# Autobot37/weatherforecastingtoolkit

Hardware: AMD Instinct MI355X
Metric: SEVIR 384x384 frames/sec (AE train step) (higher is better)
Workload: dtype f32; 1 GPU; experiments/ae_v2 conv AE (ae_64x8x8_lin.PosAwareAE_TF, img_size=384), 1x384x384 synthetic SEVIR frames, batch 32/GPU, fp32, fwd + L1 + bwd + AdamW + cosine-warmup LR; batch_per_gpu=32, global_batch=32, img_size=384, parallelism=dp1, params=215033281

## Files before the change

### include/wfae.h

```cpp
#ifndef WFAE_H
#define WFAE_H

#include <stddef.h>
#include <stdint.h>

#ifdef __cplusplus
extern "C" {
#endif

typedef void* wfae_stream_t;

typedef enum {
  WFAE_OK = 0,
  WFAE_ERR_BAD_SHAPE = -1,
  WFAE_ERR_NULL_POINTER = -2,
  WFAE_ERR_WORKSPACE = -3,
  WFAE_ERR_LAUNCH = -4,
  WFAE_ERR_UNSUPPORTED = -5
} wfae_status;

int wfae_version(void);
const char* wfae_last_error_string(void);
size_t wfae_workspace_bytes(int64_t max_weight_elems);

// ... 4 lines not shown
int wfae_set_split_gemm(int on);
int wfae_get_split_gemm(void);

int wfae_set_c1n(int on);
int wfae_get_c1n(void);

int wfae_conv1x1_fwd(const float* x, const float* w, const float* bias, const float* res,
                     int64_t res_img_stride, float* y, int NB, int Cin, int Cout, int HW,
                     wfae_stream_t stream);
int wfae_conv1x1_fwd_stats(const float* x, const float* w, const float* bias, const float* res,
                           int64_t res_img_stride, float* y, int NB, int Cin, int Cout, int HW,
                           double* stat_part, int64_t stat_capacity, int* stat_rows, wfae_stream_t stream);
int wfae_conv1x1_fwd_bnact(const float* x, const float* bn_scale, const float* bn_shift, const float* w,
                           const float* bias, const float* res, int64_t res_img_stride, float* y, int NB, int Cin,
                           int Cout, int HW, double* stat_part, int64_t stat_capacity, int* stat_rows,
                           wfae_stream_t stream);
int wfae_conv1x1_bwd_weight_bnact(const float* dy, const float* x, const float* bn_scale, const float* bn_shift,
                                  float* dw, int NB, int Cin, int Cout, int HW, int accumulate, void* ws,
                                  size_t ws_bytes, wfae_stream_t stream);
int wfae_conv1x1_bwd_data(const float* dy, const float* w, float* dx, int NB, int Cin, int Cout,
                          int HW, wfae_stream_t stream);
int wfae_conv1x1_bwd_weight(const float* dy, const float* x, float* dw, int NB, int Cin, int Cout,
                            int HW, int accumulate, void* ws, size_t ws_bytes, wfae_stream_t stream);

int wfae_c1r_supported(int M, int K, int HW);
int wfae_c1r_stat_rows(int M, int K, int NB, int HW);
int wfae_c1r_fwd(const float* w, int64_t w_sm, int64_t w_sk, const float* x, const float* pro_scale, const float* pro_shift,
                 const float* res, float* y, int NB, int K, int M, int HW, double* stat_part, int64_t stat_capacity,
                 int* stat_rows, wfae_stream_t stream);
int wfae_c1r_bnred_supported(int M, int K, int HW);
int wfae_c1r_bnred(const float* w, int64_t w_sm, int64_t w_sk, const float* dt, const float* x, const float* bn_scale,
                   const float* bn_shift, const float* save_mean, const float* save_invstd, float* da, int NB, int K, int M, int HW,
                   double* part, int64_t part_capacity, int* part_rows, wfae_stream_t stream);
int wfae_bn_act_bwd_from_rows(const double* part, int rows, int C, float* dgamma, float* dbeta, int accumulate, void* ws,
                              size_t ws_bytes, wfae_stream_t stream);
int wfae_c1r_bndx(const float* w, int64_t w_sm, int64_t w_sk, const float* dt, const float* x, const float* gamma,
                  const float* bn_scale, const float* bn_shift, const float* save_mean, const float* save_invstd, const float* coef,
                  const float* res, float* dx, int NB, int K, int M, int HW, int training, wfae_stream_t stream);
int wfae_c1rb_supported(int M, int K, int HW);
int wfae_c1rb_stat_rows(int M, int K, int NB, int HW);
int wfae_c1rb_fwd(const float* w, int64_t w_sm, int64_t w_sk, const uint16_t* x, const float* pro_scale, const float* pro_shift,
                  const uint16_t* res, uint16_t* y, int NB, int K, int M, int HW, double* stat_part, int64_t stat_capacity,
                  int* stat_rows, wfae_stream_t stream);
int wfae_c1w_supported(int Cin, int Cout, int HW);
int wfae_c1w_bwd_weight(const float* dy, const float* x, const float* bn_scale, const float* bn_shift, float* dw, int NB, int Cin,
                        int Cout, int HW, int accumulate, void* ws, size_t ws_bytes, wfae_stream_t stream);
int wfae_c1w_bwd_weight_bf16(const uint16_t* dy, const uint16_t* x, const float* bn_scale, const float* bn_shift, float* dw, int NB,
                             int Cin, int Cout, int HW, int accumulate, void* ws, size_t ws_bytes, wfae_stream_t stream);
int wfae_set_c1wd(int on);
int wfae_get_c1wd(void);
int wfae_c1wd_supported(int C, int mid, int HW);
int wfae_c1wd_bwd(const float* dy, const float* t2, const float* bn_scale, const float* bn_shift, const float* w3, float* dw3,
                  float* da3, int NB, int C, int mid, int HW, int accumulate, void* ws, size_t ws_bytes, wfae_stream_t stream);
int wfae_set_c1ws(int on);
int wfae_get_c1ws(void);
int wfae_c1ws_supported(int C, int mid, int HW);
int wfae_c1ws_stat_rows(int C, int mid, int NB, int HW, size_t ws_bytes);
int wfae_c1ws_bwd(const float* x, const float* dt1, const float* bn_scale, const float* bn_shift, const float* save_mean,
                  const float* save_invstd, const float* w1, float* dw1, double* part, int64_t part_capacity, int* part_rows, int NB,
                  int C, int mid, int HW, int accumulate, void* ws, size_t ws_bytes, wfae_stream_t stream);
int wfae_linear_fwd(const float* x, const float* w, const float* bias, float* y, int B, int In,
                    int Out, void* ws, size_t ws_bytes, wfae_stream_t stream);
int wfae_linear_bwd_data(const float* dy, const float* w, float* dx, int B, int In, int Out,
                         wfae_stream_t stream);
int wfae_linear_bwd_weight(const float* dy, const float* x, float* dw, int B, int In, int Out,
                           int accumulate, wfae_stream_t stream);
int wfae_linear_bwd_data_splitk(const float* dy, const float* w, float* dx, int B, int In, int Out, void* ws,
                                size_t ws_bytes, wfae_stream_t stream);
int wfae_linear_bwd_weight_splitk(const float* dy, const float* x, float* dw, int B, int In, int Out, int accumulate,
                                  void* ws, size_t ws_bytes, wfae_stream_t stream);

int wfae_conv4x4s2_down(const float* hi, const float* w, float* lo, int NB, int Chi, int Clo,
                        int Hlo, int Wlo, wfae_stream_t stream);
int wfae_conv4x4s2_up(const float* lo, const float* w, float* hi, int NB, int Chi, int Clo, int Hlo,
                      int Wlo, void* ws, size_t ws_bytes, wfae_stream_t stream);
int wfae_conv4x4s2_wgrad(const float* lo, const float* hi, float* dw, int NB, int Chi, int Clo,
                         int Hlo, int Wlo, int accumulate, void* ws, size_t ws_bytes,
                         wfae_stream_t stream);

int wfae_dconv_fwd(const float* x, const float* w, const float* bias, float* y, int NB, int Cin,
                   int Cout, int H, int W, int KS, int stride, int pad, int groups,
                   wfae_stream_t stream);
int wfae_dconv_bwd_data(const float* dy, const float* w, float* dx, int NB, int Cin, int Cout,
                        int H, int W, int KS, int pad, int groups, wfae_stream_t stream);
int wfae_dconv_bwd_weight(const float* dy, const float* x, float* dw, int NB, int Cin, int Cout,
                          int H, int W, int KS, int stride, int pad, int groups, int accumulate,
                          void* ws, size_t ws_bytes, wfae_stream_t stream);

int wfae_gconv3x3_fwd(const float* x, const float* w, float* y, int NB, int C, int H, int W, int groups,
                      int transposed, void* ws, size_t ws_bytes, wfae_stream_t stream);
int wfae_gconv3x3_bwd_weight(const float* dy, const float* x, float* dw, int NB, int C, int H, int W,
                             int groups, int accumulate, void* ws, size_t ws_bytes, wfae_stream_t stream);

int wfae_bn_stats_train(const float* x, int NB, int C, int HW, const float* gamma,
                        const float* beta, float eps, float momentum, float* running_mean,
                        float* running_var, float* save_mean, float* save_invstd, float* scale,
                        float* shift, void* ws, size_t ws_bytes, wfae_stream_t stream);
int wfae_bn_stats_from_rows(const double* stat_part, int rows, int NB, int C, int HW, const float* gamma,
                            const float* beta, float eps, float momentum, float* running_mean,
                            float* running_var, float* save_mean, float* save_invstd, float* scale,
                            float* shift, void* ws, size_t ws_bytes, wfae_stream_t stream);
int wfae_bn_fold_eval(const float* gamma, const float* beta, const float* running_mean,
                      const float* running_var, float eps, float* save_mean, float* save_invstd,
                      float* scale, float* shift, int C, wfae_stream_t stream);
int wfae_bn_act_fwd(const float* x, const float* scale, const float* shift, float* y, int NB, int C,
                    int HW, int act, wfae_stream_t stream);
// ... 359 lines not shown
```

### weatherforecastingtoolkit_amd/csrc/c1wd.hip

```cpp
#include "common.h"
#include <atomic>
#include <stdlib.h>
#include <type_traits>

using namespace wfae;

namespace {

typedef float f32x4 __attribute__((ext_vector_type(4)));
typedef float f32x16 __attribute__((ext_vector_type(16)));
typedef __bf16 bf16x8 __attribute__((ext_vector_type(8)));
typedef short s16x4 __attribute__((ext_vector_type(4)));
typedef short s16x8 __attribute__((ext_vector_type(8)));
typedef unsigned u32x4 __attribute__((ext_vector_type(4)));
typedef unsigned u32x2 __attribute__((ext_vector_type(2)));

struct C1WDP {
  const float* dy;
  const float* t2;
  const float* w3;
  const float* pro_scale;
  const float* pro_shift;
  float* slab;
  float* da;
  int HW;
  int cpi;
  int kc;
};

constexpr int DNT = 512, DBK = 32;

__device__ __forceinline__ unsigned off_row(int r, int c) { return (unsigned)(r * 64 + ((c ^ ((r >> 2) & 3)) << 4)); }

__device__ __forceinline__ void split_pair(float a, float b, unsigned& h, unsigned& m, unsigned& l) {
  h = pack_bf16(a, b);
  const float ra = a - bf16_lo(h), rb = b - bf16_hi(h);
  m = pack_bf16(ra, rb);
  l = pack_bf16(ra - bf16_lo(m), rb - bf16_hi(m));
}

template <int C>
__global__ __launch_bounds__(DNT, C == 128 ? 4 : 2) void c1wd_kernel(C1WDP p) {
  constexpr int M = C / 4;
  constexpr int TM = C / 128;
  constexpr int WQ = M / 32;
  constexpr int NDW = 4 * WQ;
  constexpr bool BOTH = NDW == 8;
  constexpr int KCH = C / 32;
  constexpr int LPR = 8;
  constexpr int P_LD = C * LPR, Q_LD = M * LPR;
  constexpr int P_IT = P_LD / DNT;
  static_assert(P_LD % DNT == 0 && Q_LD <= DNT, "loader");
  constexpr int A_PLANE_B = C * 64, B_PLANE_B = M * 64;
  constexpr int A_STAGE_B = 3 * A_PLANE_B, STAGE_B = 3 * (A_PLANE_B + B_PLANE_B);
  __shared__ __attribute__((aligned(16))) unsigned char smem[2 * STAGE_B];
  const int t = threadIdx.x, lane = t & 63;
  const int wave = __builtin_amdgcn_readfirstlane(t >> 6);
  const int img = blockIdx.x / p.cpi, chunk = blockIdx.x - img * p.cpi;
  const int k_begin = chunk * p.kc;
  const int k_end = min(p.HW, k_begin + p.kc);
  const int nsteps = (k_end - k_begin) / DBK;
  const bool do_dw = BOTH || wave < NDW, do_da = BOTH || wave >= NDW;

  const float* Pb = p.dy + (long)img * C * p.HW + k_begin;
  const float* Qb = p.t2 + (long)img * M * p.HW + k_begin;
  const float* p_src[P_IT];
  unsigned p_dst[P_IT];
#pragma unroll
  for (int j = 0; j < P_IT; ++j) {
    const int idx = t + j * DNT, r = idx / LPR, e = idx % LPR;
    p_src[j] = Pb + (long)r * p.HW + e * 4;
    p_dst[j] = off_row(r, e >> 1) + (unsigned)((e & 1) * 8);
  }
  const bool q_on = Q_LD == DNT || t < Q_LD;
  const int q_r = q_on ? t / LPR : 0, q_e = t % LPR;
  const float* q_src = Qb + (long)q_r * p.HW + q_e * 4;
  const unsigned q_dst = off_row(q_r, q_e >> 1) + (unsigned)((q_e & 1) * 8);
  const float q_s = p.pro_scale[q_r], q_h = p.pro_shift[q_r];
  u32x4 rp[P_IT], rq;
  auto load_global = [&]() {
#pragma unroll
    for (int j = 0; j < P_IT; ++j) rp[j] = *reinterpret_cast<const u32x4*>(p_src[j]);
    if (q_on) rq = *reinterpret_cast<const u32x4*>(q_src);
  };
  auto advance = [&](bool more) {
#pragma unroll
    for (int j = 0; j < P_IT; ++j) p_src[j] += more ? DBK : 0;
    q_src += more ? DBK : 0;
  };
  auto put = [&](unsigned char* base, int plane_b, unsigned dst, u32x4 r, bool act, float s, float h) {
    const unsigned u0 = r[0], u1 = r[1], u2 = r[2], u3 = r[3];
    float v0 = __uint_as_float(u0), v1 = __uint_as_float(u1), v2 = __uint_as_float(u2), v3 = __uint_as_float(u3);
    if (act) {
      v0 = gelu_f(fmaf(v0, s, h)); v1 = gelu_f(fmaf(v1, s, h));
      v2 = gelu_f(fmaf(v2, s, h)); v3 = gelu_f(fmaf(v3, s, h));
    }
    unsigned h0, m0, l0, h1, m1, l1;
    split_pair(v0, v1, h0, m0, l0);
    split_pair(v2, v3, h1, m1, l1);
    *reinterpret_cast<u32x2*>(base + dst) = u32x2{h0, h1};
    *reinterpret_cast<u32x2*>(base + plane_b + dst) = u32x2{m0, m1};
    *reinterpret_cast<u32x2*>(base + 2 * plane_b + dst) = u32x2{l0, l1};
  };
  auto store_lds = [&](int buf) {
    unsigned char* s = smem + buf * STAGE_B;
#pragma unroll
    for (int j = 0; j < P_IT; ++j) put(s, A_PLANE_B, p_dst[j], rp[j], false, 0.f, 0.f);
    if (q_on) put(s + A_STAGE_B, B_PLANE_B, q_dst, rq, true, q_s, q_h);
  };

  const int wm0 = (BOTH ? (wave >> 1) : (wave & 3)) * (32 * TM), wn0 = BOTH ? (wave & 1) * 32 : 0;
  const int r31 = lane & 31, lh = lane >> 5;
  const unsigned a_rd = (unsigned)((wm0 + r31) * 64), b_rd = (unsigned)((wn0 + r31) * 64);
  const int a_x = (r31 >> 2) & 3;
  f32x16 acc[TM];
  struct Frag {
    bf16x8 a[TM][3], b[3];
  };
  auto read_frag = [&](Frag& f, int buf, int ks) {
    const unsigned char* s = smem + buf * STAGE_B;
    const unsigned a_c = (unsigned)(((2 * ks + lh) ^ a_x) << 4);
#pragma unroll
    for (int i = 0; i < TM; ++i)
#pragma unroll
      for (int pl = 0; pl < 3; ++pl)
        f.a[i][pl] = *reinterpret_cast<const bf16x8*>(s + pl * A_PLANE_B + a_rd + i * (32 * 64) + a_c);
#pragma unroll
    for (int pl = 0; pl < 3; ++pl) f.b[pl] = *reinterpret_cast<const bf16x8*>(s + A_STAGE_B + pl * B_PLANE_B + b_rd + a_c);
  };
  auto mfma_frag = [&](const Frag& f) {
#pragma unroll
    for (int i = 0; i < TM; ++i) {
      f32x16 c = acc[i];
      c = __builtin_amdgcn_mfma_f32_32x32x16_bf16(f.a[i][2], f.b[0], c, 0, 0, 0);
      c = __builtin_amdgcn_mfma_f32_32x32x16_bf16(f.a[i][0], f.b[2], c, 0, 0, 0);
      c = __builtin_amdgcn_mfma_f32_32x32x16_bf16(f.a[i][1], f.b[1], c, 0, 0, 0);
      c = __builtin_amdgcn_mfma_f32_32x32x16_bf16(f.a[i][1], f.b[0], c, 0, 0, 0);
      c = __builtin_amdgcn_mfma_f32_32x32x16_bf16(f.a[i][0], f.b[1], c, 0, 0, 0);
      c = __builtin_amdgcn_mfma_f32_32x32x16_bf16(f.a[i][0], f.b[0], c, 0, 0, 0);
      acc[i] = c;
    }
  };

  const int dtile = BOTH ? wave : (wave & 3);
  const int mt = dtile >> 1, pt = dtile & 1;
  const int n16 = lane & 15, kg = lane >> 4, tq = n16 >> 2, tp = n16 & 3;
  bf16x8 wa[KCH][3];
  auto load_weights = [&]() {
#pragma unroll
    for (int ch = 0; ch < KCH; ++ch) {
      const float* src = p.w3 + (long)(32 * ch + 8 * kg) * M + 16 * mt + n16;
      float v[8];
#pragma unroll
      for (int e = 0; e < 8; ++e) v[e] = src[e * M];
      u32x4 h, m, l;
#pragma unroll
      for (int e = 0; e < 4; ++e) {
        unsigned qh, qm, ql;
        split_pair(v[2 * e], v[2 * e + 1], qh, qm, ql);
        h[e] = qh; m[e] = qm; l[e] = ql;
      }
      wa[ch][0] = __builtin_bit_cast(bf16x8, h);
      wa[ch][1] = __builtin_bit_cast(bf16x8, m);
      wa[ch][2] = __builtin_bit_cast(bf16x8, l);
    }
  };
  unsigned tr_rd[2];
#pragma unroll
  for (int hf = 0; hf < 2; ++hf) tr_rd[hf] = off_row(8 * kg + 4 * hf + tq, 2 * pt + (tp >> 1)) + 8u * (unsigned)(tp & 1);
  float* const da_dst = p.da + ((long)img * M + 16 * mt + 4 * kg) * p.HW + k_begin + 16 * pt + n16;
  auto da_step = [&](int buf, int st) {
    const unsigned char* s = smem + buf * STAGE_B;
    constexpr int PA[6] = {2, 0, 1, 1, 0, 0}, PB[6] = {0, 2, 1, 0, 1, 0};
    f32x4 d = {0.f, 0.f, 0.f, 0.f};
#pragma unroll
    for (int ch = 0; ch < KCH; ++ch) {
      bf16x8 b[3];
#pragma unroll
      for (int pl = 0; pl < 3; ++pl) {
        s16x4 part[2];
#pragma unroll
        for (int hf = 0; hf < 2; ++hf)
          part[hf] = __builtin_amdgcn_ds_read_tr16_b64_v4i16(
              (s16x4 __attribute__((address_space(3)))*)(s + pl * A_PLANE_B + ch * (32 * 64) + tr_rd[hf]));
        b[pl] = __builtin_bit_cast(bf16x8, __builtin_shufflevector(part[0], part[1], 0, 1, 2, 3, 4, 5, 6, 7));
      }
#pragma unroll
      for (int pr = 0; pr < 6; ++pr) d = __builtin_amdgcn_mfma_f32_16x16x32_bf16(wa[ch][PA[pr]], b[PB[pr]], d, 0, 0, 0);
    }
    float* o = da_dst + 32 * st;
#pragma unroll
    for (int q = 0; q < 4; ++q) o[(long)q * p.HW] = d[q];
  };

  auto run = [&](auto dwc, auto dac) {
    constexpr bool DW = decltype(dwc)::value, DA = decltype(dac)::value;
    if constexpr (DW) {
#pragma unroll
      for (int i = 0; i < TM; ++i)
#pragma unroll
        for (int q = 0; q < 16; ++q) acc[i][q] = 0.f;
    }
    if constexpr (DA) load_weights();
    if (nsteps > 0) {
      Frag f0, f1;
      load_global();
      advance(nsteps > 1);
      store_lds(0);
      load_global();
      advance(nsteps > 2);
      __syncthreads();
      if constexpr (DW) read_frag(f0, 0, 0);
      for (int st = 0; st < nsteps; ++st) {
        const int cur = st & 1;
        if constexpr (DW) read_frag(f1, cur, 1);
        store_lds(cur ^ 1);
        load_global();
        advance(st + 3 < nsteps);
        if constexpr (DW) mfma_frag(f0);
        if constexpr (DA) da_step(cur, st);
        __builtin_amdgcn_sched_barrier(0);
        __syncthreads();
        __builtin_amdgcn_sched_barrier(0);
        if constexpr (DW) {
          read_frag(f0, cur ^ 1, 0);
          mfma_frag(f1);
        }
        __builtin_amdgcn_sched_barrier(0);
      }
    }
    if constexpr (DW) {
      float* __restrict__ Cb = p.slab + (long)blockIdx.x * C * M;
#pragma unroll
      for (int i = 0; i < TM; ++i)
#pragma unroll
        for (int q = 0; q < 16; ++q) {
          const int row = wm0 + 32 * i + (q & 3) + 8 * (q >> 2) + 4 * lh;
          Cb[(long)row * M + wn0 + r31] = acc[i][q];
        }
    }
  };
  if constexpr (BOTH) run(std::true_type{}, std::true_type{});
  else if (do_dw) run(std::true_type{}, std::false_type{});
  else run(std::false_type{}, std::true_type{});
}

std::atomic<int> g_c1wd{-1};
inline bool c1wd_on() {
  int v = g_c1wd.load(std::memory_order_relaxed);
  if (v < 0) {
    const char* e = getenv("WFAE_C1WD");
    v = (e && e[0] == '0') ? 0 : 1;
    g_c1wd.store(v, std::memory_order_relaxed);
  }
  return v == 1;
}

inline bool al16(const void* q) { return (reinterpret_cast<uintptr_t>(q) & 15) == 0; }

inline bool c1wd_shape_ok(int C, int mid, int HW) { return (C == 128 || C == 256) && mid * 4 == C && HW > 0 && HW % 64 == 0; }

}

extern "C" {

int wfae_set_c1wd(int on) {
  g_c1wd.store(on ? 1 : 0, std::memory_order_relaxed);
  return WFAE_OK;
}

int wfae_get_c1wd(void) { return c1wd_on() ? 1 : 0; }

int wfae_c1wd_supported(int C, int mid, int HW) {
  return (c1wd_on() && c1wd_shape_ok(C, mid, HW) && wfae::split_gemm_enabled()) ? 1 : 0;
}

int wfae_c1wd_bwd(const float* dy, const float* t2, const float* bn_scale, const float* bn_shift, const float* w3, float* dw3,
                  float* da3, int NB, int C, int mid, int HW, int accumulate, void* ws, size_t ws_bytes, wfae_stream_t stream) {
  WFAE_REQUIRE(dy && t2 && bn_scale && bn_shift && w3 && dw3 && da3 && ws, WFAE_ERR_NULL_POINTER, "c1wd_bwd: null pointer");
  WFAE_REQUIRE(NB > 0 && C > 0 && mid > 0 && HW > 0 && NB <= 65535 && (int64_t)NB * HW < (1ll << 31), WFAE_ERR_BAD_SHAPE,
               "c1wd_bwd: bad shape");
  WFAE_REQUIRE(c1wd_shape_ok(C, mid, HW), WFAE_ERR_UNSUPPORTED,
               "c1wd_bwd: serves C = 128 or 256 with mid = C / 4 and HW %% 64 == 0 (C %d, mid %d, HW %d)", C, mid, HW);
  WFAE_REQUIRE(c1wd_on() && wfae::split_gemm_enabled(), WFAE_ERR_UNSUPPORTED,
               "c1wd_bwd: needs fp32 precision with the split GEMMs on and wfae_set_c1wd(1)");
  WFAE_REQUIRE(al16(dy) && al16(t2), WFAE_ERR_UNSUPPORTED, "c1wd_bwd: dy and t2 must be 16-byte aligned");
  C1WDP p = {};
  p.dy = dy; p.t2 = t2; p.w3 = w3;
  p.pro_scale = bn_scale; p.pro_shift = bn_shift;
  p.slab = (float*)ws; p.da = da3;
  p.HW = HW;
  WFAE_REQUIRE(c1w_chunks(C, mid, NB, HW, ws_bytes, &p.cpi, &p.kc), WFAE_ERR_WORKSPACE, "c1wd_bwd: workspace %zu < %zu", ws_bytes,
               (size_t)NB * C * mid * sizeof(float));
  hipStream_t st = (hipStream_t)stream;
  const dim3 grid((unsigned)(NB * p.cpi)), block(DNT);
  if (C == 128) hipLaunchKernelGGL((c1wd_kernel<128>), grid, block, 0, st, p);
  else hipLaunchKernelGGL((c1wd_kernel<256>), grid, block, 0, st, p);
  const int rc = check_launch("c1wd_bwd");
  if (rc) return rc;
  return slab_reduce((const float*)ws, dw3, nullptr, (long)C * mid, mid, NB * p.cpi, accumulate, st, 0);
}

}
```

### weatherforecastingtoolkit_amd/functional.py

```python
from __future__ import annotations

import os

import torch
from torch.autograd import Function

from . import ops

BN_EPS = 1e-5


_overlap = False
_side = {}


STAT_FUSION = os.environ.get("WFAE_STAT_FUSION", "1") == "1"


FUSE_A1 = os.environ.get("WFAE_FUSE_A1", "1") == "1"
FUSE_A1_MAXC = 1 << 30
FUSE_A3 = os.environ.get("WFAE_FUSE_A3", "1") == "1"
FUSE_A3_MAXC = int(os.environ.get("WFAE_FUSE_A3_MAXC", "128"))
FUSE_A3_MAXC_C1R = max(FUSE_A3_MAXC, 256)

# ... 471 lines not shown
class BottleneckFn(Function):
    @staticmethod
    def forward(ctx, x, g1, b1, w1, g2, b2, wg, g3, b3, w3, mod, x_stats=None):
        xc = _c(x)
        if xc is not x:
            x_stats = None
        x = xc
        bn1, bn2, bn3 = mod.f[0], mod.f[3], mod.f[6]
        groups = mod.f[5].groups
        training = _use_batch_stats(bn1)
        fuse = training and STAT_FUSION
        emit = fuse and getattr(mod, "emit_stats", False)
        C, mid, hw = x.shape[1], w1.shape[0], x.shape[2] * x.shape[3]
        sto = _storage(x)

        def route(op, m, k, pro=False, res="none"):
            return ops.conv1x1_route(op, m, k, hw, sto, pro, False, res)
        fused1 = FUSE_A1 and C <= FUSE_A1_MAXC and ops.conv1x1_bnact_supported(x, mid)
        r1, r3 = route("fwd", mid, C, fused1), route("fwd", C, mid, True, "ordinary")
        fused3 = (FUSE_A3 and C <= (FUSE_A3_MAXC_C1R if r3 in ("c1r", "c1rb") else FUSE_A3_MAXC)
                  and ops.conv1x1_bnact_supported((x.shape[0], mid) + x.shape[2:], C))
        if not fused3:
            r3 = route("fwd", C, mid, False, "ordinary")
        d1, d3 = (route("dgrad", C, mid), route("dgrad", mid, C)) if sto == "bf16" else (None, None)
        W1p, W3p = (ops.c1b_weights(w1), ops.c1b_weights(w3)) if "c1b" in (r1, r3, d1, d3) else ((None, None), (None, None))
        st1 = _bn_stats_rows(x_stats if (fuse or isinstance(x_stats, ops.StatParts)) else None, x, bn1, training)
        a1 = None if fused1 else ops.bn_act_fwd(x, st1, 1)
        t1, sr2 = _c1(w1, W1p[0], False, *((x, st1) if fused1 else (a1, None)), None, fuse, r1)
        st2 = _bn_stats_rows(sr2, t1, bn2, training)
        a2 = ops.bn_act_fwd(t1, st2, 1)
        t2 = _g3_fwd(a2, wg, groups)
        st3 = _bn_stats(t2, bn3, training)
        a3 = None if fused3 else ops.bn_act_fwd(t2, st3, 1)
        y, mod._out_stats = _c1(w3, W3p[0], False, *((t2, st3) if fused3 else (a3, None)), x, emit, r3)
        ctx.save_for_backward(x, _opt(a1), t1, a2, t2, _opt(a3), g1, w1, g2, wg, g3, w3,
                              st1.mean, st1.invstd, st1.scale, st1.shift,
                              st2.mean, st2.invstd, st2.scale, st2.shift,
                              st3.mean, st3.invstd, st3.scale, st3.shift,
                              _opt(W1p[1] if d1 == "c1b" else None), _opt(W3p[1] if d3 == "c1b" else None))
        ctx.training = training
        ctx.groups = groups
        ctx.betas = (b1, b2, b3)
        return y

    @staticmethod
    def backward(ctx, dy):
        (x, a1, t1, a2, t2, a3, g1, w1, g2, wg, g3, w3, *s) = ctx.saved_tensors
        st1, st2, st3 = _mk_stats(*s[0:4]), _mk_stats(*s[4:8]), _mk_stats(*s[8:12])
        W1t, W3t = s[12], s[13]
        tr = ctx.training
        dy = _c(dy)
        mid = w1.shape[0]
        dw3 = grad_buffer(w3)
        da3 = None
        if a3.numel() == 0:
            if ops.conv1x1_wd_route(dy.shape[1], mid, dy.shape[2] * dy.shape[3], _storage(dy)) == "c1wd":
                da3 = _on_main(lambda: ops.conv1x1_bwd_wd(dy, t2, st3, w3, dw3))
            if da3 is None:
                _wgrad(lambda: ops.conv1x1_bwd_weight_bnact(dy, t2, st3, dw3), dy, t2, st3.scale, st3.shift)
        else:
            _wgrad(lambda: ops.conv1x1_bwd_weight(dy, a3, dw3), dy, a3)
        dg3, db3 = grad_buffer(g3), grad_buffer(ctx.betas[2])
        if da3 is not None:
            dt2 = ops.bn_act_bwd(da3, t2, g3, st3, dg3, db3, None, 1, tr)
        else:
            dt2 = _dgrad_bn(dy, w3, W3t, t2, g3, st3, dg3, db3, None, tr)
        del da3
        dwg = grad_buffer(wg)
        _wgrad(lambda: _g3_wgrad(dt2, a2, dwg, ctx.groups), dt2, a2)
        da2 = _g3_dgrad(dt2, wg, mid, ctx.groups)
        del dt2
        dg2, db2 = grad_buffer(g2), grad_buffer(ctx.betas[1])
        dt1 = ops.bn_act_bwd(da2, t1, g2, st2, dg2, db2, None, 1, tr)
        del da2
        dw1 = grad_buffer(w1)
        rows1 = None
        if a1.numel() == 0:
            if ops.conv1x1_ws_route(x.shape[1], mid, x.shape[2] * x.shape[3], _storage(x)) == "c1ws":
                rows1 = _on_main(lambda: ops.conv1x1_bwd_ws(dt1, x, st1, w1, dw1))
            if rows1 is None:
                _wgrad(lambda: ops.conv1x1_bwd_weight_bnact(dt1, x, st1, dw1), dt1, x, st1.scale, st1.shift)
        else:
            _wgrad(lambda: ops.conv1x1_bwd_weight(dt1, a1, dw1), dt1, a1)
        dg1, db1 = grad_buffer(g1), grad_buffer(ctx.betas[0])
        dx = _dgrad_bn(dt1, w1, W1t, x, g1, st1, dg1, db1, dy, tr, rows1)
        return dx, dg1, db1, dw1, dg2, db2, dwg, dg3, db3, dw3, None, None


class Conv1x1Fn(Function):

    @staticmethod
    def forward(ctx, x, w, bias, pos):
        ctx.x_dtype = x.dtype
        x = ops.to_f32(_c(x))
        y = ops.conv1x1_fwd(x, w, bias, None if pos is None else _c(pos), pos is not None)
        ctx.save_for_backward(x, w)
        ctx.bias, ctx.pos = bias, pos
        return y

    @staticmethod
    def backward(ctx, dy):
        x, w = ctx.saved_tensors
        dy = ops.to_f32(_c(dy))
        nb, cout, h, wd = dy.shape
        dw = grad_buffer(w)
        ops.conv1x1_bwd_weight(dy, x, dw)
        dx = ops.to_dtype(ops.conv1x1_bwd_data(dy, w), ctx.x_dtype) if ctx.needs_input_grad[0] else None
        dbias = dpos = None
        if ctx.bias is not None:
            dbias = grad_buffer(ctx.bias)
            ops.reduce_sum(dy, nb, cout, h * wd, dbias)
        if ctx.pos is not None:
            dpos = grad_buffer(ctx.pos)
            ops.reduce_sum(dy, nb, cout * h * wd, 1, dpos)
        return dx, dw, dbias, dpos

# ... 1034 lines not shown
```

### weatherforecastingtoolkit_amd/ops.py

```python
from __future__ import annotations

import ctypes
import math
import os

import torch

from . import _lib

_WS_DEFAULT = int(os.environ.get("WFAE_WORKSPACE_MB", "512")) << 20
_ws = {}


def _stream():
    return torch.cuda.current_stream().cuda_stream


_prof = None


def profile_start():
    global _prof
    _prof = {}

# ... 159 lines not shown
def _p(t):
    return None if t is None else t.data_ptr()


class StatRows:
    __slots__ = ("part", "rows")

    def __init__(self, part, rows):
        self.part, self.rows = part, rows


class StatParts:
    __slots__ = ("part", "splits")

    def __init__(self, part, splits):
        self.part, self.splits = part, splits


def _rows_out(n, device):
    part = torch.empty(n, dtype=torch.float64, device=device)
    count = ctypes.c_int(0)
    return part, count, (part.data_ptr(), n, ctypes.cast(ctypes.pointer(count), ctypes.c_void_p))


_NO_ROWS = (None, 0, None)


_C1R = _C1R_BNRED = _C1R_BNDX = _C1RB = _C1B = _C1W = True


def set_c1r(on):
    global _C1R
    _C1R = bool(on)


def set_c1r_bnred(on):
    global _C1R_BNRED
    _C1R_BNRED = bool(on)


def set_c1r_bndx(on):
    global _C1R_BNDX
    _C1R_BNDX = bool(on)


def set_c1n(on):
    _lib.call("wfae_set_c1n", int(bool(on)))


def set_c1wd(on):
    _lib.call("wfae_set_c1wd", int(bool(on)))


def set_c1ws(on):
    _lib.call("wfae_set_c1ws", int(bool(on)))


def set_c1rb(on):
    global _C1RB
    _C1RB = bool(on)


def set_c1b(on):
    global _C1B
    _C1B = bool(on)


def set_c1w(on):
    global _C1W
    _C1W = bool(on)


def c1r_bndx_on():
    return _C1R_BNDX


def c1n_enabled():
    return bool(_lib.load().wfae_get_c1n())


def c1wd_enabled():
    return bool(_lib.load().wfae_get_c1wd())


def c1ws_enabled():
    return bool(_lib.load().wfae_get_c1ws())


def _precision():
    return _lib.load().wfae_get_matmul_precision()


def c1r_supported(m, k, hw):
    return _C1R and _SPLIT_GEMM and _precision() == 0 and bool(_lib.load().wfae_c1r_supported(int(m), int(k), int(hw)))


def c1r_bnred_supported(m, k, hw):
    return (_C1R and _C1R_BNRED and _SPLIT_GEMM and _precision() == 0
            and bool(_lib.load().wfae_c1r_bnred_supported(int(m), int(k), int(hw))))


def c1rb_supported(m, k, hw):
    return _C1RB and _precision() == 1 and bool(_lib.load().wfae_c1rb_supported(int(m), int(k), int(hw)))


def c1b_supported(m, k, hw):
    return _C1B and _precision() == 1 and bool(_lib.load().wfae_c1b_supported(int(m), int(k), int(hw)))


def conv1x1_bnact_supported(x, cout):
    nb, cin, h, wd = getattr(x, "shape", x)
    swapped = cin < cout and cin < 128
    return (h * wd) % 4 == 0 and h * wd >= 16 and cin % 4 == 0 and (cout % 4 == 0 or not swapped)


def conv1x1_route(op, m, k, hw, storage="f32", prologue=False, bias=False, residual="none"):
    if op == "wgrad":
        ok = _C1W and _lib.load().wfae_c1w_supported(int(k), int(m), int(hw))
        return "c1w" if ok and (_precision() == 1 if storage == "bf16" else (_precision() == 0 and _SPLIT_GEMM)) else "gemm"
    if bias or residual == "broadcast" or (residual == "ordinary" and m <= k):
        return "gemm"
    if storage == "f32":
        return "c1r" if c1r_supported(m, k, hw) else "gemm"
    rb = c1rb_supported(m, k, hw)
    if rb and not (prologue and m < k and k >= 256):
        return "c1rb"
    return "c1b" if (rb or c1b_supported(m, k, hw)) else "gemm"


def conv1x1_dgrad_bn_route(m, k, hw, storage="f32"):
    if storage == "f32" and c1r_bnred_supported(m, k, hw):
        return "bndx" if _C1R_BNDX else "bnred"
    return None


# ... 91 lines not shown
    _chk(w)
    cout, cin = w.shape[0], w.shape[1]
    Wb = torch.empty((cout, cin), dtype=BF16, device=w.device)
    Wtb = torch.empty((cin, cout), dtype=BF16, device=w.device)
    _call("wfae_c1b_weights", 0, 8 * w.numel(), _p(w), _p(Wb), _p(Wtb), cout, cin, _stream())
    return Wb, Wtb


def c1b_fwd(Wb, x, st=None, res=None, stats=False, label="wfae_c1b_fwd"):
    r = _c1_launch("c1b", Wb, False, x, st, None, res, False, stats, label)
    return r if stats else r[0]


def _c1_wgrad(dy, x, st, dw, accumulate):
    sfx, es = _chka(dy, x)
    _chk(dw)
    nb, cout, h, wd = dy.shape
    cin, n = x.shape[1], nb * h * wd
    pro = (None, None) if st is None else (_p(st.scale), _p(st.shift))
    peak = None
    if conv1x1_route("wgrad", cout, cin, h * wd, "bf16" if sfx else "f32", st is not None) == "c1w":
        name, peak = "wfae_c1w_bwd_weight" + sfx, PEAK_BF16_MFMA / (1 if sfx else 6)
    elif sfx:
        name = "wfae_conv1x1_bwd_weight_bf16"
    else:
        name, pro = ("wfae_conv1x1_bwd_weight", ()) if st is None else ("wfae_conv1x1_bwd_weight_bnact", pro)
    ws = workspace()
    _call(name, 2 * n * cin * cout, es * n * (cin + cout) + 4 * cin * cout, _p(dy), _p(x), *pro, _p(dw), nb, cin, cout, h * wd,
          int(accumulate), ws.data_ptr(), ws.numel(), _stream(), peak=peak,
          label="wfae_conv1x1_bwd_weight" if st is None else "wfae_conv1x1_bwd_weight_bnact")
    return dw


def conv1x1_bwd_weight(dy, x, dw, accumulate=False):
    return _c1_wgrad(dy, x, None, dw, accumulate)


def conv1x1_bwd_weight_bnact(dy, x, st, dw, accumulate=False):
    return _c1_wgrad(dy, x, st, dw, accumulate)


C1WD_MIN_HW = 512


def conv1x1_wd_supported(c, mid, hw, storage="f32"):
    return (storage == "f32" and _SPLIT_GEMM and _precision() == 0 and bool(_lib.load().wfae_c1wd_supported(int(c), int(mid), int(hw)))
            and conv1x1_route("wgrad", c, mid, hw, "f32", True) == "c1w" and conv1x1_route("dgrad", mid, c, hw) == "c1r")


def conv1x1_wd_route(c, mid, hw, storage="f32"):
    return "c1wd" if hw >= C1WD_MIN_HW and conv1x1_wd_supported(c, mid, hw, storage) else "pair"


def conv1x1_bwd_wd(dy, t2, st, w3, dw3, accumulate=False):
    if st is None or dy.dtype != torch.float32 or t2.dtype != torch.float32:
        return None
    nb, c, h, wd = dy.shape
    mid, hw = t2.shape[1], h * wd
    if not conv1x1_wd_supported(c, mid, hw):
        return None
    _chk(dy, t2, w3, dw3)
    if tuple(t2.shape) != (nb, mid, h, wd) or w3.numel() != c * mid or dw3.numel() != c * mid:
        raise _lib.WfaeError("conv1x1_bwd_wd: dy (N, C, H, W), t2 (N, C/4, H, W), w3 and dw3 (C, C/4)")
    if (dy.data_ptr() | t2.data_ptr()) & 15:
        return None
    da = torch.empty_like(t2)
    n = nb * hw
    ws = workspace()
    _call("wfae_c1wd_bwd", 4 * n * c * mid, 4 * n * (c + 2 * mid) + 8 * c * mid, _p(dy), _p(t2), _p(st.scale), _p(st.shift), _p(w3),
          _p(dw3), _p(da), nb, c, mid, hw, int(accumulate), ws.data_ptr(), ws.numel(), _stream(), peak=PEAK_BF16_MFMA / 6,
          label="wfae_c1wd_bwd")
    return da


def conv1x1_ws_supported(c, mid, hw, storage="f32"):
    return (storage == "f32" and _SPLIT_GEMM and _precision() == 0 and bool(_lib.load().wfae_c1ws_supported(int(c), int(mid), int(hw)))
            and conv1x1_route("wgrad", mid, c, hw, "f32", True) == "c1w" and conv1x1_dgrad_bn_route(c, mid, hw, storage) == "bndx")


def conv1x1_ws_route(c, mid, hw, storage="f32"):
    return "c1ws" if hw >= C1WD_MIN_HW and conv1x1_ws_supported(c, mid, hw, storage) else "pair"


def conv1x1_bwd_ws(dt1, x, st, w1, dw1, accumulate=False):
    if st is None or dt1.dtype != torch.float32 or x.dtype != torch.float32:
        return None
    nb, c, h, wd = x.shape
    mid, hw = dt1.shape[1], h * wd
    if not conv1x1_ws_supported(c, mid, hw):
        return None
    _chk(dt1, x, w1, dw1)
    if tuple(dt1.shape) != (nb, mid, h, wd) or w1.numel() != c * mid or dw1.numel() != c * mid:
        raise _lib.WfaeError("conv1x1_bwd_ws: x (N, C, H, W), dt1 (N, C/4, H, W), w1 and dw1 (C/4, C)")
    if (dt1.data_ptr() | x.data_ptr()) & 15:
        return None
    n = nb * hw
    ws = workspace()
    cap = 2 * int(_lib.load().wfae_c1ws_stat_rows(c, mid, nb, hw, ws.numel())) * c
    if cap <= 0:
        return None
    part, rows, out = _rows_out(cap, x.device)
    _call("wfae_c1ws_bwd", 4 * n * c * mid, 4 * n * (c + mid) + 8 * c * mid, _p(x), _p(dt1), _p(st.scale), _p(st.shift), _p(st.mean),
          _p(st.invstd), _p(w1), _p(dw1), *out, nb, c, mid, hw, int(accumulate), ws.data_ptr(), ws.numel(), _stream(),
          peak=PEAK_BF16_MFMA / 6, label="wfae_c1ws_bwd")
    return StatRows(part[:2 * rows.value * c], rows.value)


def c1r_bnred(w, dt, x, st, store=True):
    _chk(w, dt, x)
    nb, k, h, wd = dt.shape
    m, n = w.shape[1], nb * h * wd
    da = torch.empty((nb, m, h, wd), dtype=torch.float32, device=dt.device) if store else None
    part, rows, out = _rows_out(2 * int(_lib.load().wfae_c1r_stat_rows(m, k, nb, h * wd)) * m, dt.device)
    _call("wfae_c1r_bnred", 2 * n * k * m, 4 * (n * (k + (2 if store else 1) * m) + k * m), _p(w), 1, m, _p(dt), _p(x), _p(st.scale),
          _p(st.shift), _p(st.mean), _p(st.invstd), _p(da), nb, k, m, h * wd, *out, _stream(), label="wfae_conv1x1_bwd_data",
          peak=_C1_PEAK["c1r"])
    return da, StatRows(part[:2 * rows.value * m], rows.value)


def bn_act_bwd_from_rows(sr, c, dgamma, dbeta, accumulate=False):
    _chk(dgamma, dbeta)
# ... 1996 lines not shown
```

Before: 181.7 frames/s.

## Fuse BN-backward channel sums into the c1wd dgrad/wgrad kernel

Adds a SUMS variant of the fused conv1x1 weight/data-gradient kernel. While producing da3 it also computes the per-channel sums of da*gelu'(bn(x)) and da*gelu'*xhat in double precision and writes them as partial rows. The BN backward can then take dgamma/dbeta from those rows and run only the dx pass, which avoids a separate reduction that rereads da3 and t2. The cost is extra LDS, wave-local syncs, a reordered load/store pipeline in the da waves, and a block-wide barrier at the end. The path is on by default through an env flag and applies only when mid*hw reaches a threshold.

```diff
diff --git a/include/wfae.h b/include/wfae.h
--- a/include/wfae.h
+++ b/include/wfae.h
@@ -80,6 +80,13 @@
 int wfae_c1wd_supported(int C, int mid, int HW);
 int wfae_c1wd_bwd(const float* dy, const float* t2, const float* bn_scale, const float* bn_shift, const float* w3, float* dw3,
                   float* da3, int NB, int C, int mid, int HW, int accumulate, void* ws, size_t ws_bytes, wfae_stream_t stream);
+int wfae_set_c1wd_sums(int on);
+int wfae_get_c1wd_sums(void);
+int wfae_c1wd_stat_rows(int C, int mid, int NB, int HW, size_t ws_bytes);
+int wfae_c1wd_bwd_sums(const float* dy, const float* t2, const float* bn_scale, const float* bn_shift, const float* save_mean,
+                       const float* save_invstd, const float* w3, float* dw3, float* da3, double* part, int64_t part_capacity,
+                       int* part_rows, int NB, int C, int mid, int HW, int accumulate, void* ws, size_t ws_bytes,
+                       wfae_stream_t stream);
 int wfae_set_c1ws(int on);
 int wfae_get_c1ws(void);
 int wfae_c1ws_supported(int C, int mid, int HW);
diff --git a/weatherforecastingtoolkit_amd/csrc/c1wd.hip b/weatherforecastingtoolkit_amd/csrc/c1wd.hip
--- a/weatherforecastingtoolkit_amd/csrc/c1wd.hip
+++ b/weatherforecastingtoolkit_amd/csrc/c1wd.hip
@@ -21,14 +21,20 @@
   const float* w3;
   const float* pro_scale;
   const float* pro_shift;
+  const float* mean;
+  const float* invstd;
   float* slab;
   float* da;
+  double* part0;
+  double* part1;
   int HW;
   int cpi;
   int kc;
 };
 
 constexpr int DNT = 512, DBK = 32;
+constexpr int X_LD = 20;
+constexpr int X_TILE_B = 16 * X_LD * 4, X_WAVE_B = X_TILE_B + 2 * 64 * 16;
 
 __device__ __forceinline__ unsigned off_row(int r, int c) { return (unsigned)(r * 64 + ((c ^ ((r >> 2) & 3)) << 4)); }
 
@@ -39,7 +45,7 @@
   l = pack_bf16(ra - bf16_lo(m), rb - bf16_hi(m));
 }
 
-template <int C>
+template <int C, bool SUMS>
 __global__ __launch_bounds__(DNT, C == 128 ? 4 : 2) void c1wd_kernel(C1WDP p) {
   constexpr int M = C / 4;
   constexpr int TM = C / 128;
@@ -53,7 +59,9 @@
   static_assert(P_LD % DNT == 0 && Q_LD <= DNT, "loader");
   constexpr int A_PLANE_B = C * 64, B_PLANE_B = M * 64;
   constexpr int A_STAGE_B = 3 * A_PLANE_B, STAGE_B = 3 * (A_PLANE_B + B_PLANE_B);
-  __shared__ __attribute__((aligned(16))) unsigned char smem[2 * STAGE_B];
+  constexpr int NDA = M / 8;
+  static_assert(2 * STAGE_B + NDA * X_WAVE_B <= (C == 128 ? 78 : 156) * 1024, "LDS");
+  __shared__ __attribute__((aligned(16))) unsigned char smem[2 * STAGE_B + (SUMS ? NDA * X_WAVE_B : 0)];
   const int t = threadIdx.x, lane = t & 63;
   const int wave = __builtin_amdgcn_readfirstlane(t >> 6);
   const int img = blockIdx.x / p.cpi, chunk = blockIdx.x - img * p.cpi;
@@ -61,6 +69,8 @@
   const int k_end = min(p.HW, k_begin + p.kc);
   const int nsteps = (k_end - k_begin) / DBK;
   const bool do_dw = BOTH || wave < NDW, do_da = BOTH || wave >= NDW;
+  const int dtile = BOTH ? wave : (wave & 3);
+  const int mt = dtile >> 1, pt = dtile & 1;
 
   const float* Pb = p.dy + (long)img * C * p.HW + k_begin;
   const float* Qb = p.t2 + (long)img * M * p.HW + k_begin;
@@ -72,16 +82,22 @@
     p_src[j] = Pb + (long)r * p.HW + e * 4;
     p_dst[j] = off_row(r, e >> 1) + (unsigned)((e & 1) * 8);
   }
-  const bool q_on = Q_LD == DNT || t < Q_LD;
-  const int q_r = q_on ? t / LPR : 0, q_e = t % LPR;
+  const bool q_on = SUMS ? do_da : (Q_LD == DNT || t < Q_LD);
+  const int q_r = !q_on ? 0 : SUMS ? 16 * mt + (lane >> 2) : t / LPR, q_e = SUMS ? 4 * pt + (lane & 3) : t % LPR;
   const float* q_src = Qb + (long)q_r * p.HW + q_e * 4;
   const unsigned q_dst = off_row(q_r, q_e >> 1) + (unsigned)((q_e & 1) * 8);
   const float q_s = p.pro_scale[q_r], q_h = p.pro_shift[q_r];
   u32x4 rp[P_IT], rq;
+  auto load_p = [&]() {
+#pragma unroll
+    for (int j = 0; j < P_IT; ++j) rp[j] = *reinterpret_cast<const u32x4*>(p_src[j]);
+  };
+  auto load_q = [&]() {
+    if (q_on) rq = *reinterpret_cast<const u32x4*>(q_src);
+  };
   auto load_global = [&]() {
-#pragma unroll
-    for (int j = 0; j < P_IT; ++j) rp[j] = *reinterpret_cast<const u32x4*>(p_src[j]);
-    if (q_on) rq = *reinterpret_cast<const u32x4*>(q_src);
+    load_p();
+    load_q();
   };
   auto advance = [&](bool more) {
 #pragma unroll
@@ -102,11 +118,42 @@
     *reinterpret_cast<u32x2*>(base + plane_b + dst) = u32x2{m0, m1};
     *reinterpret_cast<u32x2*>(base + 2 * plane_b + dst) = u32x2{l0, l1};
   };
+  auto store_p = [&](int buf) {
+    unsigned char* s = smem + buf * STAGE_B;
+#pragma unroll
+    for (int j = 0; j < P_IT; ++j) put(s, A_PLANE_B, p_dst[j], rp[j], false, 0.f, 0.f);
+  };
+  unsigned char* const xt = smem + 2 * STAGE_B + (SUMS ? dtile * X_WAVE_B : 0);
+  unsigned char* const park = xt + X_TILE_B + lane * 16;
+  float q_mu = 0.f, q_is = 0.f;
+  if constexpr (SUMS) {
+    q_mu = p.mean[q_r];
+    q_is = p.invstd[q_r];
+  }
+  double sum1 = 0.0, sum2 = 0.0;
+  auto store_q = [&](int buf) {
+    unsigned char* s = smem + buf * STAGE_B + A_STAGE_B;
+    if constexpr (SUMS) {
+      if (q_on) {
+        const unsigned u0 = rq[0], u1 = rq[1], u2 = rq[2], u3 = rq[3];
+        const float x0 = __uint_as_float(u0), x1 = __uint_as_float(u1), x2 = __uint_as_float(u2), x3 = __uint_as_float(u3);
+        const float w0 = fmaf(x0, q_s, q_h), w1 = fmaf(x1, q_s, q_h), w2 = fmaf(x2, q_s, q_h), w3 = fmaf(x3, q_s, q_h);
+        *reinterpret_cast<f32x4*>(park) = f32x4{gelu_grad_f(w0), gelu_grad_f(w1), gelu_grad_f(w2), gelu_grad_f(w3)};
+        *reinterpret_cast<f32x4*>(park + 1024) = f32x4{(x0 - q_mu) * q_is, (x1 - q_mu) * q_is, (x2 - q_mu) * q_is, (x3 - q_mu) * q_is};
+        unsigned h0, m0, l0, h1, m1, l1;
+        split_pair(gelu_f(w0), gelu_f(w1), h0, m0, l0);
+        split_pair(gelu_f(w2), gelu_f(w3), h1, m1, l1);
+        *reinterpret_cast<u32x2*>(s + q_dst) = u32x2{h0, h1};
+        *reinterpret_cast<u32x2*>(s + B_PLANE_B + q_dst) = u32x2{m0, m1};
+        *reinterpret_cast<u32x2*>(s + 2 * B_PLANE_B + q_dst) = u32x2{l0, l1};
+      }
+    } else {
+      if (q_on) put(s, B_PLANE_B, q_dst, rq, true, q_s, q_h);
+    }
+  };
   auto store_lds = [&](int buf) {
-    unsigned char* s = smem + buf * STAGE_B;
-#pragma unroll
-    for (int j = 0; j < P_IT; ++j) put(s, A_PLANE_B, p_dst[j], rp[j], false, 0.f, 0.f);
-    if (q_on) put(s + A_STAGE_B, B_PLANE_B, q_dst, rq, true, q_s, q_h);
+    store_p(buf);
+    store_q(buf);
   };
 
   const int wm0 = (BOTH ? (wave >> 1) : (wave & 3)) * (32 * TM), wn0 = BOTH ? (wave & 1) * 32 : 0;
@@ -142,8 +189,6 @@
     }
   };
 
-  const int dtile = BOTH ? wave : (wave & 3);
-  const int mt = dtile >> 1, pt = dtile & 1;
   const int n16 = lane & 15, kg = lane >> 4, tq = n16 >> 2, tp = n16 & 3;
   bf16x8 wa[KCH][3];
   auto load_weights = [&]() {
@@ -191,6 +236,25 @@
     float* o = da_dst + 32 * st;
 #pragma unroll
     for (int q = 0; q < 4; ++q) o[(long)q * p.HW] = d[q];
+    if constexpr (SUMS) {
+      float* const x_wr = reinterpret_cast<float*>(xt) + (4 * kg) * X_LD + n16;
+#pragma unroll
+      for (int q = 0; q < 4; ++q) x_wr[q * X_LD] = d[q];
+      __builtin_amdgcn_fence(__ATOMIC_RELEASE, "wavefront");
+      __builtin_amdgcn_wave_barrier();
+      __builtin_amdgcn_fence(__ATOMIC_ACQUIRE, "wavefront");
+      const f32x4 v = *reinterpret_cast<const f32x4*>(xt + ((lane >> 2) * X_LD + 4 * (lane & 3)) * 4);
+      const f32x4 g = *reinterpret_cast<const f32x4*>(park), xh = *reinterpret_cast<const f32x4*>(park + 1024);
+      const float d0 = v.x * g.x, d1 = v.y * g.y;
+      const float d2 = v.z * g.z, d3 = v.w * g.w;
+      const float h0 = xh.x, h1 = xh.y, h2 = xh.z, h3 = xh.w;
+      const float s1 = (d0 + d1) + (d2 + d3);
+      const float s2 = fmaf(d0, h0, d1 * h1) + fmaf(d2, h2, d3 * h3);
+      sum1 += (double)s1;
+      sum2 += (double)s2;
+      __builtin_amdgcn_fence(__ATOMIC_RELEASE, "wavefront");
+      __builtin_amdgcn_wave_barrier();
+    }
   };
 
   auto run = [&](auto dwc, auto dac) {
@@ -214,11 +278,21 @@
       for (int st = 0; st < nsteps; ++st) {
         const int cur = st & 1;
         if constexpr (DW) read_frag(f1, cur, 1);
-        store_lds(cur ^ 1);
-        load_global();
-        advance(st + 3 < nsteps);
-        if constexpr (DW) mfma_frag(f0);
-        if constexpr (DA) da_step(cur, st);
+        if constexpr (SUMS && DA) {
+          store_p(cur ^ 1);
+          load_p();
+          if constexpr (DW) mfma_frag(f0);
+          da_step(cur, st);
+          store_q(cur ^ 1);
+          load_q();
+          advance(st + 3 < nsteps);
+        } else {
+          store_lds(cur ^ 1);
+          load_global();
+          advance(st + 3 < nsteps);
+          if constexpr (DW) mfma_frag(f0);
+          if constexpr (DA) da_step(cur, st);
+        }
         __builtin_amdgcn_sched_barrier(0);
         __syncthreads();
         __builtin_amdgcn_sched_barrier(0);
@@ -243,6 +317,29 @@
   if constexpr (BOTH) run(std::true_type{}, std::true_type{});
   else if (do_dw) run(std::true_type{}, std::false_type{});
   else run(std::false_type{}, std::true_type{});
+
+  if constexpr (SUMS) {
+    double e1 = sum1, e2 = sum2;
+    double* const mine = reinterpret_cast<double*>(xt) + 2 * (lane >> 2);
+    if (do_da) {
+#pragma unroll
+      for (int o = 1; o < 4; o <<= 1) {
+        e1 += __shfl_xor(e1, o, 64);
+        e2 += __shfl_xor(e2, o, 64);
+      }
+      if (pt == 1 && (lane & 3) == 0) {
+        mine[0] = e1;
+        mine[1] = e2;
+      }
+    }
+    __syncthreads();
+    if (do_da && pt == 0 && (lane & 3) == 0) {
+      const double* other = reinterpret_cast<const double*>(xt + X_WAVE_B) + 2 * (lane >> 2);
+      const long at = (long)blockIdx.x * M + 16 * mt + (lane >> 2);
+      p.part0[at] = e1 + other[0];
+      p.part1[at] = e2 + other[1];
+    }
+  }
 }
 
 std::atomic<int> g_c1wd{-1};
@@ -256,9 +353,60 @@
   return v == 1;
 }
 
+std::atomic<int> g_c1wd_sums{-1};
+inline bool c1wd_sums_on() {
+  int v = g_c1wd_sums.load(std::memory_order_relaxed);
+  if (v < 0) {
+    const char* e = getenv("WFAE_C1WD_SUMS");
+    v = (e && e[0] == '0') ? 0 : 1;
+    g_c1wd_sums.store(v, std::memory_order_relaxed);
+  }
+  return v == 1;
+}
+
 inline bool al16(const void* q) { return (reinterpret_cast<uintptr_t>(q) & 15) == 0; }
 
 inline bool c1wd_shape_ok(int C, int mid, int HW) { return (C == 128 || C == 256) && mid * 4 == C && HW > 0 && HW % 64 == 0; }
+
+int c1wd_launch(const char* what, const float* dy, const float* t2, const float* bn_scale, const float* bn_shift,
+                const float* save_mean, const float* save_invstd, const float* w3, float* dw3, float* da3, double* part,
+                int64_t part_capacity, int* part_rows, int NB, int C, int mid, int HW, int accumulate, void* ws, size_t ws_bytes,
+                wfae_stream_t stream) {
+  const bool sums = part != nullptr;
+  WFAE_REQUIRE(dy && t2 && bn_scale && bn_shift && w3 && dw3 && da3 && ws, WFAE_ERR_NULL_POINTER, "%s: null pointer", what);
+  WFAE_REQUIRE(NB > 0 && C > 0 && mid > 0 && HW > 0 && NB <= 65535 && (int64_t)NB * HW < (1ll << 31), WFAE_ERR_BAD_SHAPE,
+               "%s: bad shape", what);
+  WFAE_REQUIRE(c1wd_shape_ok(C, mid, HW), WFAE_ERR_UNSUPPORTED,
+               "%s: serves C = 128 or 256 with mid = C / 4 and HW %% 64 == 0 (C %d, mid %d, HW %d)", what, C, mid, HW);
+  WFAE_REQUIRE(c1wd_on() && wfae::split_gemm_enabled(), WFAE_ERR_UNSUPPORTED,
+               "%s: needs fp32 precision with the split GEMMs on and wfae_set_c1wd(1)", what);
+  WFAE_REQUIRE(!sums || c1wd_sums_on(), WFAE_ERR_UNSUPPORTED, "%s: needs wfae_set_c1wd_sums(1)", what);
+  WFAE_REQUIRE(al16(dy) && al16(t2), WFAE_ERR_UNSUPPORTED, "%s: dy and t2 must be 16-byte aligned", what);
+  C1WDP p = {};
+  p.dy = dy; p.t2 = t2; p.w3 = w3;
+  p.pro_scale = bn_scale; p.pro_shift = bn_shift; p.mean = save_mean; p.invstd = save_invstd;
+  p.slab = (float*)ws; p.da = da3;
+  p.HW = HW;
+  WFAE_REQUIRE(c1w_chunks(C, mid, NB, HW, ws_bytes, &p.cpi, &p.kc), WFAE_ERR_WORKSPACE, "%s: workspace %zu < %zu", what, ws_bytes,
+               (size_t)NB * C * mid * sizeof(float));
+  const int rows = NB * p.cpi;
+  if (sums) {
+    WFAE_REQUIRE(part_capacity >= 2 * (int64_t)rows * mid, WFAE_ERR_WORKSPACE, "%s: part holds %lld doubles, needs %lld", what,
+                 (long long)part_capacity, (long long)(2 * (int64_t)rows * mid));
+    *part_rows = rows;
+    p.part0 = part;
+    p.part1 = part + (long)rows * mid;
+  }
+  hipStream_t st = (hipStream_t)stream;
+  const dim3 grid((unsigned)rows), block(DNT);
+  if (C == 128 && sums) hipLaunchKernelGGL((c1wd_kernel<128, true>), grid, block, 0, st, p);
+  else if (C == 128) hipLaunchKernelGGL((c1wd_kernel<128, false>), grid, block, 0, st, p);
+  else if (sums) hipLaunchKernelGGL((c1wd_kernel<256, true>), grid, block, 0, st, p);
+  else hipLaunchKernelGGL((c1wd_kernel<256, false>), grid, block, 0, st, p);
+  const int rc = check_launch(what);
+  if (rc) return rc;
+  return slab_reduce((const float*)ws, dw3, nullptr, (long)C * mid, mid, rows, accumulate, st, 0);
+}
 
 }
 
@@ -275,30 +423,32 @@
   return (c1wd_on() && c1wd_shape_ok(C, mid, HW) && wfae::split_gemm_enabled()) ? 1 : 0;
 }
 
+int wfae_set_c1wd_sums(int on) {
+  g_c1wd_sums.store(on ? 1 : 0, std::memory_order_relaxed);
+  return WFAE_OK;
+}
+
+int wfae_get_c1wd_sums(void) { return c1wd_sums_on() ? 1 : 0; }
+
+int wfae_c1wd_stat_rows(int C, int mid, int NB, int HW, size_t ws_bytes) {
+  int cpi = 0, kc = 0;
+  if (!c1wd_shape_ok(C, mid, HW) || NB <= 0 || !c1w_chunks(C, mid, NB, HW, ws_bytes, &cpi, &kc)) return 0;
+  return NB * cpi;
+}
+
 int wfae_c1wd_bwd(const float* dy, const float* t2, const float* bn_scale, const float* bn_shift, const float* w3, float* dw3,
                   float* da3, int NB, int C, int mid, int HW, int accumulate, void* ws, size_t ws_bytes, wfae_stream_t stream) {
-  WFAE_REQUIRE(dy && t2 && bn_scale && bn_shift && w3 && dw3 && da3 && ws, WFAE_ERR_NULL_POINTER, "c1wd_bwd: null pointer");
-  WFAE_REQUIRE(NB > 0 && C > 0 && mid > 0 && HW > 0 && NB <= 65535 && (int64_t)NB * HW < (1ll << 31), WFAE_ERR_BAD_SHAPE,
-               "c1wd_bwd: bad shape");
-  WFAE_REQUIRE(c1wd_shape_ok(C, mid, HW), WFAE_ERR_UNSUPPORTED,
-               "c1wd_bwd: serves C = 128 or 256 with mid = C / 4 and HW %% 64 == 0 (C %d, mid %d, HW %d)", C, mid, HW);
-  WFAE_REQUIRE(c1wd_on() && wfae::split_gemm_enabled(), WFAE_ERR_UNSUPPORTED,
-               "c1wd_bwd: needs fp32 precision with the split GEMMs on and wfae_set_c1wd(1)");
-  WFAE_REQUIRE(al16(dy) && al16(t2), WFAE_ERR_UNSUPPORTED, "c1wd_bwd: dy and t2 must be 16-byte aligned");
-  C1WDP p = {};
-  p.dy = dy; p.t2 = t2; p.w3 = w3;
-  p.pro_scale = bn_scale; p.pro_shift = bn_shift;
-  p.slab = (float*)ws; p.da = da3;
-  p.HW = HW;
-  WFAE_REQUIRE(c1w_chunks(C, mid, NB, HW, ws_bytes, &p.cpi, &p.kc), WFAE_ERR_WORKSPACE, "c1wd_bwd: workspace %zu < %zu", ws_bytes,
-               (size_t)NB * C * mid * sizeof(float));
-  hipStream_t st = (hipStream_t)stream;
-  const dim3 grid((unsigned)(NB * p.cpi)), block(DNT);
-  if (C == 128) hipLaunchKernelGGL((c1wd_kernel<128>), grid, block, 0, st, p);
-  else hipLaunchKernelGGL((c1wd_kernel<256>), grid, block, 0, st, p);
-  const int rc = check_launch("c1wd_bwd");
-  if (rc) return rc;
-  return slab_reduce((const float*)ws, dw3, nullptr, (long)C * mid, mid, NB * p.cpi, accumulate, st, 0);
-}
-
-}
+  return c1wd_launch("c1wd_bwd", dy, t2, bn_scale, bn_shift, nullptr, nullptr, w3, dw3, da3, nullptr, 0, nullptr, NB, C, mid, HW,
+                     accumulate, ws, ws_bytes, stream);
+}
+
+int wfae_c1wd_bwd_sums(const float* dy, const float* t2, const float* bn_scale, const float* bn_shift, const float* save_mean,
+                       const float* save_invstd, const float* w3, float* dw3, float* da3, double* part, int64_t part_capacity,
+                       int* part_rows, int NB, int C, int mid, int HW, int accumulate, void* ws, size_t ws_bytes,
+                       wfae_stream_t stream) {
+  WFAE_REQUIRE(save_mean && save_invstd && part && part_rows, WFAE_ERR_NULL_POINTER, "c1wd_bwd_sums: null pointer");
+  return c1wd_launch("c1wd_bwd_sums", dy, t2, bn_scale, bn_shift, save_mean, save_invstd, w3, dw3, da3, part, part_capacity, part_rows,
+                     NB, C, mid, HW, accumulate, ws, ws_bytes, stream);
+}
+
+}
diff --git a/weatherforecastingtoolkit_amd/functional.py b/weatherforecastingtoolkit_amd/functional.py
--- a/weatherforecastingtoolkit_amd/functional.py
+++ b/weatherforecastingtoolkit_amd/functional.py
@@ -547,16 +547,24 @@
         dy = _c(dy)
         mid = w1.shape[0]
         dw3 = grad_buffer(w3)
-        da3 = None
+        da3 = rows3 = None
         if a3.numel() == 0:
             if ops.conv1x1_wd_route(dy.shape[1], mid, dy.shape[2] * dy.shape[3], _storage(dy)) == "c1wd":
-                da3 = _on_main(lambda: ops.conv1x1_bwd_wd(dy, t2, st3, w3, dw3))
+                if ops.conv1x1_wd_sums_route(dy.shape[1], mid, dy.shape[2] * dy.shape[3], _storage(dy)) == "sums":
+                    both = _on_main(lambda: ops.conv1x1_bwd_wd(dy, t2, st3, w3, dw3, sums=True))
+                    if both is not None:
+                        da3, rows3 = both
+                if da3 is None:
+                    da3 = _on_main(lambda: ops.conv1x1_bwd_wd(dy, t2, st3, w3, dw3))
             if da3 is None:
                 _wgrad(lambda: ops.conv1x1_bwd_weight_bnact(dy, t2, st3, dw3), dy, t2, st3.scale, st3.shift)
         else:
             _wgrad(lambda: ops.conv1x1_bwd_weight(dy, a3, dw3), dy, a3)
         dg3, db3 = grad_buffer(g3), grad_buffer(ctx.betas[2])
-        if da3 is not None:
+        if rows3 is not None:
+            ops.bn_act_bwd_from_rows(rows3, mid, dg3, db3)
+            dt2 = ops.bn_act_bwd_dx(da3, t2, g3, st3, None, 1, tr)
+        elif da3 is not None:
             dt2 = ops.bn_act_bwd(da3, t2, g3, st3, dg3, db3, None, 1, tr)
         else:
             dt2 = _dgrad_bn(dy, w3, W3t, t2, g3, st3, dg3, db3, None, tr)
diff --git a/weatherforecastingtoolkit_amd/ops.py b/weatherforecastingtoolkit_amd/ops.py
--- a/weatherforecastingtoolkit_amd/ops.py
+++ b/weatherforecastingtoolkit_amd/ops.py
@@ -235,6 +235,10 @@
     _lib.call("wfae_set_c1wd", int(bool(on)))
 
 
+def set_c1wd_sums(on):
+    _lib.call("wfae_set_c1wd_sums", int(bool(on)))
+
+
 def set_c1ws(on):
     _lib.call("wfae_set_c1ws", int(bool(on)))
 
@@ -264,6 +268,10 @@
 
 def c1wd_enabled():
     return bool(_lib.load().wfae_get_c1wd())
+
+
+def c1wd_sums_enabled():
+    return bool(_lib.load().wfae_get_c1wd_sums())
 
 
 def c1ws_enabled():
@@ -461,12 +469,20 @@
     return "c1wd" if hw >= C1WD_MIN_HW and conv1x1_wd_supported(c, mid, hw, storage) else "pair"
 
 
-def conv1x1_bwd_wd(dy, t2, st, w3, dw3, accumulate=False):
+C1WD_SUMS_MIN_T2 = 1 << 20
+
+
+def conv1x1_wd_sums_route(c, mid, hw, storage="f32"):
+    return ("sums" if c1wd_sums_enabled() and mid * hw >= C1WD_SUMS_MIN_T2 and conv1x1_wd_route(c, mid, hw, storage) == "c1wd"
+            else "reduce")
+
+
+def conv1x1_bwd_wd(dy, t2, st, w3, dw3, accumulate=False, sums=False):
     if st is None or dy.dtype != torch.float32 or t2.dtype != torch.float32:
         return None
     nb, c, h, wd = dy.shape
     mid, hw = t2.shape[1], h * wd
-    if not conv1x1_wd_supported(c, mid, hw):
+    if not conv1x1_wd_supported(c, mid, hw) or (sums and not c1wd_sums_enabled()):
         return None
     _chk(dy, t2, w3, dw3)
     if tuple(t2.shape) != (nb, mid, h, wd) or w3.numel() != c * mid or dw3.numel() != c * mid:
@@ -476,6 +492,15 @@
     da = torch.empty_like(t2)
     n = nb * hw
     ws = workspace()
+    if sums:
+        cap = 2 * int(_lib.load().wfae_c1wd_stat_rows(c, mid, nb, hw, ws.numel())) * mid
+        if cap <= 0:
+            return None
+        part, rows, out = _rows_out(cap, dy.device)
+        _call("wfae_c1wd_bwd_sums", 4 * n * c * mid, 4 * n * (c + 2 * mid) + 8 * c * mid, _p(dy), _p(t2), _p(st.scale), _p(st.shift),
+              _p(st.mean), _p(st.invstd), _p(w3), _p(dw3), _p(da), *out, nb, c, mid, hw, int(accumulate), ws.data_ptr(), ws.numel(),
+              _stream(), peak=PEAK_BF16_MFMA / 6, label="wfae_c1wd_bwd")
+        return da, StatRows(part[:2 * rows.value * mid], rows.value)
     _call("wfae_c1wd_bwd", 4 * n * c * mid, 4 * n * (c + 2 * mid) + 8 * c * mid, _p(dy), _p(t2), _p(st.scale), _p(st.shift), _p(w3),
           _p(dw3), _p(da), nb, c, mid, hw, int(accumulate), ws.data_ptr(), ws.numel(), _stream(), peak=PEAK_BF16_MFMA / 6,
           label="wfae_c1wd_bwd")
```

After: 182.9 frames/s, median of 6. Within noise of the previous version (+0.6%).
